# Bismarrck/tensoralloy

Hardware: AMD Instinct MI355X
Metric: atom-steps/sec (energy+forces), 4000-atom Ni rcut=6.5 A (higher is better)
Workload: dtype f64

## Files before the change

tensoralloy_amd/csrc/ta_api.hip:

```cpp
#include <hip/hip_runtime.h>

#include <algorithm>
#include <chrono>
#include <climits>
#include <cmath>
#include <cstdio>
#include <cstdlib>
#include <cstring>
#include <stdexcept>
#include <string>
#include <vector>

#include "ta_device.h"
#include "ta_internal.h"
#include "ta_md.h"
#include "ta_neb.h"
#include "ta_relax.h"

namespace ta {
size_t mlp_scratch_doubles(const MlpDev &mlp);
void launch_mlp_impl(const MlpDev &mlp, int activation, int ndim, const int32_t *atoms, int n_atoms,
                     const DeviceBatch &b, const Options &opt, double *scratch, hipStream_t s,
                     MlpLaunchInfo *info = nullptr);
size_t mlp_all_scratch_doubles(const MlpDev *mlps_host, int nel, const int32_t *elem_start);
// ... 204 lines not shown
  double rmax = 0.0;
  ta::SFParams sf;
  std::vector<ChunkPlan> chunks;
  std::vector<ChunkPlan> chunks_v2;
  bool use_v2 = false;
  ta::MlpDev *mlp_dev = nullptr;
  ta::MlpDev mlp[ta::kMaxElements];
  bool td = false, td_sommerfeld = false;
  int td_act = 0, td_K = 0;
  ta::MlpDev td_nets[3 * ta::kMaxElements];
  ta::MlpDev *td_dev = nullptr;
  std::vector<void *> model_allocs;
  ta::EamModel *eam = nullptr;
  ta::GrapModel *grap = nullptr;

  ta::HostPairs hp;
  ta::DeviceBatch db;
  bool have_batch = false;
  uint32_t last_want = 0;

  PinnedBuf stage_in, stage_out;
  DevBuf<char> inbuf;
  DevBuf<double> results;
  size_t o_blk = 0;
  int res_n_blk = 0;
  DevBuf<double> rec, part4, G, dEdG, g, wat, bpart, fown, benergy, mlp_scratch;
  DevBuf<double> td_T, td_u, td_s;
  DevBuf<unsigned long long> masks;
  DevBuf<uint32_t> job_word;
  DevBuf<int32_t> job_count;
  DevBuf<uint32_t> job_word_own;
  DevBuf<int32_t> job_count_own;
  bool triangles = true;
  bool tri_cells_ok = false;
  bool tri_cells_wide_ok = false;
  int last_bwd_variant = 0;
  ta::MlpLaunchInfo last_mlp_launch;
  DevBuf<int32_t> pair_start, seg_start, pair_i, pair_j, pair_shift, pair_rev;
  ta::NlGrid *d_grids = nullptr;
  DevBuf<int32_t> nl_wrap, nl_binid, nl_bin_count, nl_bin_start, nl_bin_cursor, nl_bin_atoms, nl_counts;
  DevBuf<unsigned long long> nl_stats, nl_zero;
  unsigned long long *nl_stats_ptr = nullptr;
  bool nl_sorted = false;
  bool nl_rev_done = false;
  bool nl_zero_clean = false;
  int64_t nl_zero_atoms = -1;
  int nl_zero_bins = -1;
  DevBuf<double> hvp_buf;
#ifdef TA_PHASE_STAMPS
  DevBuf<unsigned long long> stamp_buf;
#endif
  DevBuf<ta::NlRec> nl_recs;
  bool pairs_on_device = false;
  bool descriptors_valid = false;
  DevBuf<double> train_scratch, train_partial, train_grad, train_coeff;
  DevBuf<double> jvp_J, tan_dD, tan_dG, tan_dir;
  DevBuf<double> filt_scratch;
  bool jvp_valid = false;

  double skin = 0.0;
  double r_list = 0.0;
  std::vector<int32_t> keep_species;
  std::vector<int32_t> keep_natoms, keep_pbc;
  std::vector<double> ref_pos, ref_cells;
  size_t o_pos = 0, o_cells = 0, o_species = 0;
  DevBuf<int32_t> ex_pair_i, ex_pair_j, ex_pair_shift, ex_pair_rev, ex_pair_start, ex_pair_stop, ex_seg_start, ex_counts,
// ... 513 lines not shown
}

#ifdef TA_PHASE_STAMPS
static void dump_stamps(ta_context *h) {
  const std::string &path = h->opt.phase_stamps_out;
  if (path.empty() || !h->db.stamps || h->db.n_blk <= 0) return;
  const size_t n = (size_t)2 * h->db.n_blk * ta::kStampSlots;
  std::vector<unsigned long long> v(n);
  (void)hipStreamSynchronize(h->stream);
  (void)hipMemcpy(v.data(), h->db.stamps, n * sizeof(unsigned long long), hipMemcpyDeviceToHost);
  FILE *fp = std::fopen(path.c_str(), "w");
  if (!fp) return;
  for (int k = 0; k < 2; ++k)
    for (int b = 0; b < h->db.n_blk; ++b) {
      std::fprintf(fp, "%d %d", k, b);
      for (int q = 0; q < ta::kStampSlots; ++q)
        std::fprintf(fp, " %llu", v[((size_t)k * h->db.n_blk + b) * ta::kStampSlots + q]);
      std::fprintf(fp, "\n");
    }
  std::fclose(fp);
}
#endif

void launch_head(ta_context *h, const ta::DeviceBatch &db, hipStream_t s) {
  if (h->td)
    ta::launch_td_all(h->td_dev, h->td_nets, h->n_elements, h->td_K, h->td_act, h->activation,
                      h->td_sommerfeld ? 1 : 0, h->sf.ndim, db, h->opt.mlp_da_global, h->td_T.ptr, h->td_u.ptr, h->td_s.ptr,
                      h->mlp_scratch.ptr, s, &h->last_mlp_launch);
  else
    ta::launch_mlp_all(h->mlp_dev, h->mlp, h->n_elements, h->activation, h->sf.ndim, db, h->opt, h->mlp_scratch.ptr,
                       s, &h->last_mlp_launch);
}

void compute_impl(ta_context *h, uint32_t want, bool timed, double *slot_ms) {
  using namespace ta;
#ifdef TA_PHASE_STAMPS
  if (h->db.n_blk > 0) {
    h->stamp_buf.ensure((size_t)2 * h->db.n_blk * ta::kStampSlots + 8);
    h->db.stamps = h->stamp_buf.ptr;
    (void)hipMemsetAsync(h->db.stamps, 0, (size_t)2 * h->db.n_blk * ta::kStampSlots * sizeof(unsigned long long),
                         h->stream);
  }
#endif
  h->db.rec4 = nullptr;
  h->db.own_sums = 0;
  const DeviceBatch &db = h->db;
  hipStream_t s = h->stream;
  const bool need_forces = (want & (TA_WANT_FORCES | TA_WANT_VIRIAL)) != 0;
  auto begin = [&](int slot) {
    if (timed) HIP_CHECK(hipEventRecord(h->ev[2 * slot], s));
  };
  auto end = [&](int slot) {
    if (timed) HIP_CHECK(hipEventRecord(h->ev[2 * slot + 1], s));
  };
  bool used[TA_N_KERNEL_SLOTS] = {false};

  const bool has_mlp = h->kind == TA_MODEL_SF_MLP || h->kind == TA_MODEL_GRAP_MLP;
  if ((want & TA_WANT_REUSE_DESCRIPTORS) && has_mlp && h->descriptors_valid && !need_forces) {
    begin(TA_K_MLP);
    launch_head(h, db, s);
    end(TA_K_MLP);
    used[TA_K_MLP] = true;
  } else if (h->kind == TA_MODEL_SF_MLP) {
    h->db.rec4 = (h->sf.angular && h->use_v2 && !h->opt.full_records) ? h->db.rec : nullptr;
    if (!h->use_v2) {
      begin(TA_K_PAIR_GEOMETRY);
      launch_pair_geometry(h->sf, db, s);
      end(TA_K_PAIR_GEOMETRY);
      used[TA_K_PAIR_GEOMETRY] = true;
    }
    h->sf.ang_scale = h->use_v2 ? 1.0 : 0.5;
    const bool tri_cells = (h->relax_cell_on || h->md_baro_on) ? h->tri_cells_wide_ok : h->tri_cells_ok;
    const bool tri = h->use_v2 && h->triangles && tri_cells && h->n_elements == 1 && need_forces;
    h->db.job_word_own = (tri && h->db.job_count) ? h->job_word_own.ptr : nullptr;
    h->db.job_count_own = (tri && h->db.job_count) ? h->job_count_own.ptr : nullptr;
    h->last_bwd_variant = 0;
    const bool reduce_in_forward = h->sf.angular && h->use_v2;
    if (h->sf.angular) {
      begin(TA_K_G4_FORWARD);
      if (h->use_v2) {
        bool geometry = true;
        size_t left = h->chunks_v2.size();
        for (const ChunkPlan &cp : h->chunks_v2) {
          --left;
          launch_g4_forward_v2(h->sf, cp.ch, cp.ng, cp.nz, geometry, left == 0, db, h->opt, s);
          geometry = false;
        }
      } else
        for (const ChunkPlan &cp : h->chunks) launch_g4_forward(h->sf, cp.ch, cp.nb, cp.ng, cp.nz, db, s);
      end(TA_K_G4_FORWARD);
      used[TA_K_G4_FORWARD] = true;
    }
    if (!reduce_in_forward) {
      begin(TA_K_DESCRIPTOR_REDUCE);
      launch_descriptor_reduce(h->sf, db, s);
      end(TA_K_DESCRIPTOR_REDUCE);
      used[TA_K_DESCRIPTOR_REDUCE] = true;
    }
    begin(TA_K_MLP);
    launch_head(h, db, s);
    end(TA_K_MLP);
    used[TA_K_MLP] = true;
    if (need_forces) {
      begin(TA_K_BACKWARD);
      if (h->sf.angular) {
        bool first = true;
        if (h->use_v2)
          for (const ChunkPlan &cp : h->chunks_v2) {
            h->last_bwd_variant |= launch_backward_v2(h->sf, cp.ch, cp.ng, cp.nz, first, tri, db, h->opt, s);
            first = false;
          }
        else
          for (const ChunkPlan &cp : h->chunks) {
            launch_backward(h->sf, cp.ch, cp.nb, cp.ng, cp.nz, first, false, db, s);
            first = false;
          }
      } else {
        AngChunk dummy;
        std::memset(&dummy, 0, sizeof(dummy));
        launch_backward(h->sf, dummy, 1, 1, 1, true, true, db, s);
      }
// ... 283 lines not shown
  h->filtered = true;
}

bool cells_admit_triangles(double rmax, int32_t n_frames, const ta_frame *frames) {
  for (int f = 0; f < n_frames; ++f) {
    const double *c = frames[f].cell;
    const double vol = std::fabs(c[0] * (c[4] * c[8] - c[5] * c[7]) - c[1] * (c[3] * c[8] - c[5] * c[6]) +
                                 c[2] * (c[3] * c[7] - c[4] * c[6]));
    for (int k = 0; k < 3; ++k) {
      if (!frames[f].pbc[k]) continue;
      const double *u = c + 3 * ((k + 1) % 3), *v = c + 3 * ((k + 2) % 3);
      const double nx = u[1] * v[2] - u[2] * v[1], ny = u[2] * v[0] - u[0] * v[2], nz = u[0] * v[1] - u[1] * v[0];
      const double area = std::sqrt(nx * nx + ny * ny + nz * nz);
      if (!(vol > rmax * area)) return false;
    }
  }
  return true;
}

void set_frames_impl(ta_context *h, int32_t n_frames, const ta_frame *frames, ta_batch_info *info) {
  for (int f = 0; f < n_frames; ++f) {
    const ta_frame &fr = frames[f];
    if (fr.n_atoms < 0 || (fr.n_atoms > 0 && (!fr.species || !fr.positions)) || !fr.cell || !fr.pbc)
      throw std::invalid_argument("frame " + std::to_string(f) + ": null array");
  }
  const auto t_begin = std::chrono::steady_clock::now();
  if (h->upload_pending) {
    HIP_CHECK(hipStreamSynchronize(h->stream));
    h->upload_pending = false;
  }
  h->have_batch = false;
  h->descriptors_valid = false;
  h->jvp_valid = false;
  h->mirror_want = 0;
  h->filtered = false;
  h->db.slot_q = h->db.rev_super = h->db.rev_map = nullptr;
  h->db.pair_stop = nullptr;
  h->db.blk_groups = 0;
  h->db.n_blk_dev = nullptr;
  h->r_list = h->rmax + h->skin;
  h->tri_cells_ok = cells_admit_triangles(h->rmax, n_frames, frames);
  h->tri_cells_wide_ok = cells_admit_triangles(h->r_list, n_frames, frames);
  size_t N = 0;
  for (int f = 0; f < n_frames; ++f) N += (size_t)frames[f].n_atoms;
  if (N >= (1u << 30)) throw std::runtime_error("batch too large for 32-bit atom indices");
  const size_t F = (size_t)n_frames;
  const int nel = h->n_elements;
  auto align16 = [](size_t x) { return (x + 15) & ~(size_t)15; };
  const size_t o_pos = 0;
  const size_t o_cells = align16(o_pos + 3 * N * sizeof(double));
  const size_t o_grids = align16(o_cells + 9 * F * sizeof(double));
  const size_t o_species = align16(o_grids + F * sizeof(ta::NlGrid));
  const size_t o_foa = align16(o_species + N * sizeof(int32_t));
  const size_t o_astart = align16(o_foa + N * sizeof(int32_t));
  const size_t o_elem = align16(o_astart + (F + 1) * sizeof(int32_t));
  const size_t o_blk = align16(o_elem + N * sizeof(int32_t));
  auto align64 = [](size_t x) { return (x + 63) & ~(size_t)63; };
  const size_t total = align64(o_blk + (N + 2) * sizeof(int32_t)) + (N + 1) * sizeof(ta::BlockHeader);
  h->stage_in.ensure(total);
  h->inbuf.ensure(total);
  char *hb = h->stage_in.ptr;
  double *pos = reinterpret_cast<double *>(hb + o_pos);
  double *cells = reinterpret_cast<double *>(hb + o_cells);
  ta::NlGrid *grids = reinterpret_cast<ta::NlGrid *>(hb + o_grids);
  int32_t *species = reinterpret_cast<int32_t *>(hb + o_species);
  int32_t *foa = reinterpret_cast<int32_t *>(hb + o_foa);
// ... 252 lines not shown
}

int ta_set_skin(ta_handle h, double skin) {
  if (!h) return TA_ERR_INVALID;
  if (!(skin >= 0.0) || !std::isfinite(skin)) return fail(h, TA_ERR_INVALID, "skin must be a finite length >= 0");
  if (skin != h->skin) {
    h->skin = skin;
    h->have_batch = false;
    h->descriptors_valid = false;
  }
  return TA_OK;
}

int ta_update_positions(ta_handle h, const double *positions, const double *cells, int32_t *rebuilt) {
  if (!h || !positions) return fail(h, TA_ERR_INVALID, "null argument");
  if (h->ref_pos.empty() && h->keep_natoms.empty())
    return fail(h, TA_ERR_INVALID, "ta_update_positions called before ta_set_frames");
  return guarded(h, [&]() {
    const size_t N = h->keep_species.size(), F = h->keep_natoms.size();
    bool keep = h->have_batch && h->skin > 0.0;
    if (keep && cells) keep = std::memcmp(cells, h->ref_cells.data(), 9 * F * sizeof(double)) == 0;
    if (keep) {
      if (h->upload_pending) {
        HIP_CHECK(hipStreamSynchronize(h->stream));
        h->upload_pending = false;
      }
      double *stage = reinterpret_cast<double *>(h->stage_in.ptr + h->o_pos);
      std::memcpy(stage, positions, 3 * N * sizeof(double));
      staged_copy(h->db.pos, stage, 3 * N, false, h->opt, h->stream);
      h->upload_pending = true;
      if (h->filtered) apply_filter(h);
      h->descriptors_valid = false;
      h->jvp_valid = false;
      const double lim2 = 0.25 * h->skin * h->skin;
      const double *ref = h->ref_pos.data();
      for (size_t i = 0; i < N; ++i) {
        const double dx = positions[3 * i] - ref[3 * i], dy = positions[3 * i + 1] - ref[3 * i + 1],
                     dz = positions[3 * i + 2] - ref[3 * i + 2];
        const double d2 = dx * dx + dy * dy + dz * dz;
        if (!(d2 <= lim2)) {
          keep = false;
          break;
        }
      }
    }
    if (rebuilt) *rebuilt = keep ? 0 : 1;
    if (keep) {
      ++h->n_list_reuses;
      return;
    }
    rebuild_list(h, positions, cells);
    if (cells && h->relax_cell_on && h->relax_valid && F) {
      HIP_CHECK(hipMemcpy(h->relax_cell_h0.ptr, h->ref_cells.data(), 9 * F * sizeof(double), hipMemcpyHostToDevice));
      h->relax_cell_G_host.assign(9 * F, 0.0);
      for (size_t f = 0; f < F; ++f) h->relax_cell_G_host[9 * f] = h->relax_cell_G_host[9 * f + 4] = h->relax_cell_G_host[9 * f + 8] = 1.0;
      h->relax_cell_vel_host.assign(9 * F, 0.0);
    }
  });
}

int ta_list_stats(ta_handle h, int64_t *n_builds, int64_t *n_reuses) {
  if (!h) return TA_ERR_INVALID;
  if (n_builds) *n_builds = h->n_list_builds;
  if (n_reuses) *n_reuses = h->n_list_reuses;
  return TA_OK;
}
// ... 1311 lines not shown
    size_t scratch = 0, partial = 0;
    for (int e = 0; e < h->n_elements; ++e) {
      const int n_el = h->db.elem_start[e + 1] - h->db.elem_start[e];
      scratch = std::max(scratch, ta::mlp_grad_scratch_doubles(h->mlp[e], n_el));
      partial = std::max(partial, ta::mlp_grad_partial_doubles(h->mlp[e], n_el));
    }
    h->train_scratch.ensure(scratch + 8);
    h->train_partial.ensure(partial + 8);
    h->train_grad.ensure((size_t)total + 8);
    h->train_coeff.ensure(F + 8);
    if (F) HIP_CHECK(hipMemcpyAsync(h->train_coeff.ptr, frame_coeff, F * sizeof(double), hipMemcpyHostToDevice, s));
    size_t off = 0;
    for (int e = 0; e < h->n_elements; ++e) {
      const int n_el = h->db.elem_start[e + 1] - h->db.elem_start[e];
      ta::launch_mlp_grad(h->mlp[e], h->activation, h->sf.ndim, h->db.elem_atoms + h->db.elem_start[e], n_el,
                          h->db, h->train_coeff.ptr, h->train_scratch.ptr, h->train_partial.ptr,
                          h->train_grad.ptr + off, s);
      off += (size_t)ta::mlp_param_count(h->mlp[e]);
    }
    HIP_CHECK(hipGetLastError());
    HIP_CHECK(hipMemcpyAsync(grad, h->train_grad.ptr, (size_t)total * sizeof(double), hipMemcpyDeviceToHost, s));
    HIP_CHECK(hipStreamSynchronize(s));
  });
}

namespace {
void backward_only(ta_context *h) {
  using namespace ta;
  const DeviceBatch &db = h->db;
  hipStream_t s = h->stream;
  if (h->kind == TA_MODEL_SF_MLP) {
    if (h->sf.angular) {
      bool first = true;
      if (h->use_v2)
        for (const ChunkPlan &cp : h->chunks_v2) {
          launch_backward_v2(h->sf, cp.ch, cp.ng, cp.nz, first, false, db, h->opt, s);
          first = false;
        }
      else
        for (const ChunkPlan &cp : h->chunks) {
          launch_backward(h->sf, cp.ch, cp.nb, cp.ng, cp.nz, first, false, db, s);
          first = false;
        }
    } else {
      AngChunk dummy;
      std::memset(&dummy, 0, sizeof(dummy));
      launch_backward(h->sf, dummy, 1, 1, 1, true, true, db, s);
    }
  } else {
    launch_grap_backward(h->grap, db, s);
  }
}
void ensure_pair_jacobians(ta_context *h) {
  hipStream_t s = h->stream;
  const size_t N = (size_t)h->db.n_atoms, P = (size_t)h->db.n_pairs;
  const int D = h->sf.ndim;
  if (!h->descriptors_valid || !h->jvp_valid)
    compute_impl(h, TA_WANT_ENERGY, false, nullptr);
  if (h->jvp_valid) return;
  h->jvp_J.ensure((size_t)D * 4 * P + 8);
  for (int c = 0; c < D; ++c) {
    ta::launch_one_hot(h->db.dEdG, (int64_t)N, D, c, s);
    backward_only(h);
    if (P)
      HIP_CHECK(hipMemcpyAsync(h->jvp_J.ptr + (size_t)c * 4 * P, h->db.g, 4 * P * sizeof(double),
                               hipMemcpyDeviceToDevice, s));
  }
  HIP_CHECK(hipGetLastError());
  h->jvp_valid = true;
}
}

// ... 703 lines not shown
```

tensoralloy_amd/csrc/ta_device.h:

```cpp
#pragma once
#include <hip/hip_runtime.h>

#include <cstdint>
#include <type_traits>

#include "ta_options.h"
#include "tensoralloy_amd.h"

namespace ta {

constexpr int kMaxRadial = 64;
constexpr int kMaxElements = 8;
constexpr int kMaxBetaSlots = 3;
constexpr int kRecDoubles = 8;
constexpr int kMaxLayers = 8;
constexpr int kCapMin = 192;
constexpr int kCapMax = 1024;
constexpr int kMaxCentersPerBlock = 16;
constexpr int kMaxHd = 24;
constexpr int kStampSlots = 10;

struct SFParams {
  double rcut, acut;
  double inv_rc2, inv_ac2;
// ... 117 lines not shown
  int32_t ndim;
  uint32_t stride_nrad;
};
static_assert(sizeof(LaunchHead) == 64 && alignof(LaunchHead) == 64, "one line of the argument segment");
static_assert(std::is_trivially_copyable<LaunchHead>::value && std::is_standard_layout<LaunchHead>::value,
              "passed by value in the argument segment");
static_assert(4 * kCapMax < (1 << 16) && kMaxRadial < (1 << 8), "job_stride and n_rad share a word");

__host__ __device__ inline int triangle_owner_rank(uint32_t index_sum) {
#ifdef __HIP_DEVICE_COMPILE__
  const uint32_t h = __umul24(index_sum, 0x9E3779u);
#else
  const uint32_t h = index_sum * 0x9E3779u;
#endif
  return (int)(((h & 0xFFFFFFu) * 3u) >> 24);
}
__host__ __device__ inline bool owns_triangle(int32_t i, int32_t j, int32_t k) {
  return triangle_owner_rank((uint32_t)i + (uint32_t)j + (uint32_t)k) == (j < i ? 1 : 0) + (k < i ? 1 : 0);
}

#ifdef __HIPCC__
__device__ __forceinline__ int pair_stop_of(const DeviceBatch &b, int64_t i) {
  return b.pair_stop ? b.pair_stop[i] : b.pair_start[i + 1];
}
#endif

#ifdef __HIPCC__
__device__ __forceinline__ int pair_rev_of(const DeviceBatch &b, int q) {
  return b.slot_q ? b.rev_map[b.rev_super[b.slot_q[q]]] : b.pair_rev[q];
}
__device__ __forceinline__ const double2 *pair_geom(const DeviceBatch &b, size_t q) {
  return reinterpret_cast<const double2 *>(b.rec4 ? b.rec4 + 4 * q : b.rec + kRecDoubles * q);
}
#endif

struct MlpLayerDev {
  int k, n;
  int kp, np;
  double *w;
  double *wt;
  double *b;
  int act;
  int res;
};
struct MlpDev {
  int n_layers = 0;
  MlpLayerDev layer[kMaxLayers];
  double *xlo = nullptr, *xhi = nullptr;
  int max_np = 0, max_kp = 0;
};

struct MlpLaunchInfo {
  int family = 0;
  int threads = 0;
  int lh = 0;
  int nt = 0;
  int grid_x = 0, grid_y = 0;
  long long lds_bytes = 0;
  int da = 0;
};

void launch_pair_geometry(const SFParams &sf, const DeviceBatch &b, hipStream_t s);
void launch_g4_forward(const SFParams &sf, const AngChunk &ch, int nb, int ng, int nz,
                       const DeviceBatch &b, hipStream_t s);
void launch_descriptor_reduce(const SFParams &sf, const DeviceBatch &b, hipStream_t s);
void launch_mlp(const SFParams &sf, const MlpDev &mlp, int activation, int element,
                const DeviceBatch &b, hipStream_t s);
void launch_backward(const SFParams &sf, const AngChunk &ch, int nb, int ng, int nz,
                     bool first, bool radial_only, const DeviceBatch &b, hipStream_t s);
void launch_force_gather(const SFParams &sf, const DeviceBatch &b, int gather_w, hipStream_t s);
void launch_frame_reduce(const DeviceBatch &b, bool want_virial, double *mirror, int64_t n_tail, hipStream_t s);

size_t g4_lds_bytes(int nnl_max);

size_t v2_lds_bytes(bool backward, int cap, int n_local = 0, int nspec = 0, bool triangles = false);
int v2_job_stride(int cap);
void launch_g4_forward_v2(const SFParams &sf, const AngChunk &ch, int ng, int nz, bool geometry,
                          bool reduce, const DeviceBatch &b, const Options &opt, hipStream_t s);
int launch_backward_v2(const SFParams &sf, const AngChunk &ch, int ng, int nz, bool first, bool triangles,
                       const DeviceBatch &b, const Options &opt, hipStream_t s);

struct NlGrid {
  double h[9];
  double hinv[9];
  double lo[3];
  double inv_w[3];
  int32_t nb[3];
  int32_t pbc[3];
  int32_t bin_offset;
  int32_t pad_;
  int32_t m[3];
  int32_t ortho;
  double bw[3];
};
struct NlRec {
  double x, y, z;
  int32_t wx, wy, wz;
  int32_t j;
  int32_t sp;
  int32_t pad_;
};
struct NlWork {
  int32_t *wrap;
  int32_t *binid;
  int32_t *bin_count;
  int32_t *bin_start;
  int32_t *bin_cursor;
  int32_t *bin_atoms;
  NlRec *recs;
  int32_t *counts;
  int32_t *seg_start;
// ... 29 lines not shown
```

tensoralloy_amd/csrc/ta_kernels_v2.hip:

```cpp
#include <hip/hip_runtime.h>

#include <cstdio>
#include <cstdlib>
#include <stdexcept>
#include <type_traits>

#include "ta_device.h"
#include "ta_math.h"
#include "ta_reduce.h"

namespace ta {
namespace {

constexpr int kBlock = 256;
constexpr int kNF = 8;
constexpr int kNFf = 7;
constexpr int kSegW = 6;
constexpr int kOwnCtl = 60 + 2 * kMaxCentersPerBlock * kSegW;
constexpr int kJobCtlBytes = (kOwnCtl + 40) * 4;
__host__ __device__ inline int v2_pcols(int cap, int nspec) {
  return nspec >= 1 ? cap / 4 + kMaxCentersPerBlock * nspec : cap;
}
constexpr int kRingPad = 64;
constexpr int kRTab = 8;

#ifdef TA_LDS_PROBE
__device__ __forceinline__ bool kProbe(int flags, int bit) { return (flags >> bit) & 1; }
#else
__device__ __forceinline__ constexpr bool kProbe(int, int) { return false; }
#endif

#ifdef TA_PHASE_STAMPS
#define TA_STAMP(b, kernel, k)                                                                          \
  do {                                                                                                  \
    if ((b).stamps && threadIdx.x == 0)                                                                 \
      (b).stamps[((size_t)(kernel) * gridDim.x + blockIdx.x) * kStampSlots + (k)] = __builtin_amdgcn_s_memrealtime(); \
  } while (0)
#define TA_STAMP_ENTRY() const unsigned long long ta_t_start_ = __builtin_amdgcn_s_memrealtime()
#define TA_STAMP_HEADER(b, kernel, hd)                                                                  \
  do {                                                                                                  \
    if ((b).stamps && threadIdx.x == 0 && (hd).M >= 0) {                                                \
      unsigned long long *dst_ = (b).stamps + ((size_t)(kernel) * gridDim.x + blockIdx.x) * kStampSlots; \
      dst_[9] = __builtin_amdgcn_s_memrealtime();                                                       \
      dst_[8] = ta_t_start_;                                                                            \
    }                                                                                                   \
  } while (0)
#else
#define TA_STAMP(b, kernel, k) do {} while (0)
#define TA_STAMP_ENTRY() do {} while (0)
#define TA_STAMP_HEADER(b, kernel, hd) do {} while (0)
#endif

__device__ __forceinline__ void pin_head(const LaunchHead &h) {
  asm volatile("" ::"s"(h.blk_hdr), "s"(h.n_blk_dev), "s"(h.job_count), "s"(h.job_word), "s"(h.dEdG),
               "s"(h.pair_j), "s"(h.blk_groups), "s"(h.flags), "s"(h.ndim), "s"(h.stride_nrad));
// ... 94 lines not shown
  if constexpr (HD > 0) {
    double p = ch.hd[HD - 1], d = 0.0;
#pragma unroll
    for (int k = HD - 2; k >= 0; --k) {
      d = fma(d, u, p);
      p = fma(p, u, ch.hd[k]);
    }
    h = p;
    dh = d;
  } else {
    double fd, dfd;
    cutoff_u(sf.cutoff, u, fd, dfd);
    const double ed = ta_exp(-beta * u);
    h = ed * fd;
    dh = ed * (dfd - beta * fd);
  }
}
template <int HD>
__device__ __forceinline__ double hd_value(const SFParams &sf, const AngChunk &ch, double beta,
                                           double u) {
  if constexpr (HD > 0) {
    double p = ch.hd[HD - 1];
#pragma unroll
    for (int k = HD - 2; k >= 0; --k) p = fma(p, u, ch.hd[k]);
    return p;
  } else {
    return ta_exp(-beta * u) * cutoff_u_value(sf.cutoff, u);
  }
}

template <int HD>
__device__ __forceinline__ void stage(const SFParams &sf, const AngChunk &ch, double beta, const DeviceBatch &b,
                                      const Fields &f, const HeaderRegs &hd, const int32_t *pair_j, bool one_el,
                                      unsigned nthr, int geom = 0, bool forward = false, int *jidx = nullptr) {
  const int s0 = hd.s0, M = hd.M;
  for (int item = threadIdx.x; item < M; item += nthr) {
    double2 v0, v1, v2;
    int ci = 0, cbase = 0, cn = 0;
    if (geom || forward) centre_of(hd, item, ci, cbase, cn);
    const bool want_j = geom || jidx || !one_el;
    const int j = want_j ? (pair_j ? pair_j : b.pair_j)[s0 + item] : 0;
    const double spj = one_el ? 0.0 : (double)b.species[j];
    if (geom) {
      const int64_t p = (int64_t)s0 + item;
      const int i = hd.c0 + ci;
      const double *h = b.cells + 9 * (size_t)b.frame_of_atom[i];
      const double sx = (double)b.pair_shift[3 * p], sy = (double)b.pair_shift[3 * p + 1],
                   sz = (double)b.pair_shift[3 * p + 2];
      const double *ri = b.pos + 3 * (size_t)i, *rj = b.pos + 3 * (size_t)j;
      const double dx = (rj[0] - ri[0]) + (sx * h[0] + sy * h[3] + sz * h[6]);
      const double dy = (rj[1] - ri[1]) + (sx * h[1] + sy * h[4] + sz * h[7]);
      const double dz = (rj[2] - ri[2]) + (sx * h[2] + sy * h[5] + sz * h[8]);
      const double r2 = dx * dx + dy * dy + dz * dz + sf.eps;
      v0 = make_double2(dx, dy);
      v1 = make_double2(dz, r2);
      v2 = make_double2(1.0 / sqrt(r2), 0.0);
      if (b.rec4) {
        double2 *dst = reinterpret_cast<double2 *>(b.rec4 + 4 * (size_t)p);
        dst[0] = v0;
        dst[1] = v1;
      } else {
        double2 *dst = reinterpret_cast<double2 *>(b.rec + kRecDoubles * (size_t)p);
        dst[0] = v0;
        dst[1] = v1;
        dst[2] = v2;
        dst[3] = make_double2(0.0, 0.0);
      }
    } else if (b.rec4) {
      const double2 *src = reinterpret_cast<const double2 *>(b.rec4 + 4 * (size_t)(s0 + item));
      v0 = src[0];
      v1 = src[1];
      v2 = make_double2(1.0 / sqrt(v1.y), 0.0);
    } else {
      const double2 *src = reinterpret_cast<const double2 *>(b.rec + kRecDoubles * (size_t)(s0 + item));
      v0 = src[0];
      v1 = src[1];
      v2 = src[2];
    }
    f.xy[item] = v0;
    f.zr[item] = v1;
    if (forward) {
      const int k0 = 2 * cbase + (item - cbase);
      f.xf[k0] = f.xf[k0 + cn] = (float)v0.x;
      f.yf[k0] = f.yf[k0 + cn] = (float)v0.y;
      f.zf[k0] = f.zf[k0 + cn] = (float)v1.x;
    }
    const double u = v1.y * sf.inv_ac2;
    double H = 0.0, L = 0.0;
    if (u < 1.0) {
      if (forward) {
        H = hd_value<HD>(sf, ch, beta, u);
      } else {
        double dH;
        hd_eval<HD>(sf, ch, beta, u, H, dH);
        L = (H != 0.0) ? sf.two_inv_ac2 * dH / H : 0.0;
      }
    }
    f.ih[item] = make_double2(v2.x, H);
    if (jidx) jidx[item] = j;
    else if (forward) f.sp1[item] = spj;
    else f.gs[item] = make_double2(L, spj);
  }
  __syncthreads();
}

__device__ __forceinline__ unsigned long long partner_mask(const SFParams &sf, const Fields &f,
                                                           int base, int n, int a, int sc, int smax) {
  const int ring = 2 * base + a;
  const float ax = f.xf[ring], ay = f.yf[ring], az = f.zf[ring];
  const float lim = (float)(sf.acut * sf.acut) * 1.0001f;
  unsigned long long mask = 0ull;
  const int count = smax - sc + 1;
  typedef float f32x2 __attribute__((ext_vector_type(2)));
  const f32x2 ax2 = {ax, ax}, ay2 = {ay, ay}, az2 = {az, az};
  for (int g = 0; g < 4 && 16 * g < count; ++g) {
    const float *px = f.xf + ring + sc + 16 * g, *py = f.yf + ring + sc + 16 * g,
                *pz = f.zf + ring + sc + 16 * g;
    unsigned m = 0u;
#pragma unroll
    for (int k = 14; k >= 0; k -= 2) {
      const f32x2 vx = {px[k], px[k + 1]}, vy = {py[k], py[k + 1]}, vz = {pz[k], pz[k + 1]};
      const f32x2 ex = vx - ax2, ey = vy - ay2, ez = vz - az2;
      const f32x2 d2 = __builtin_elementwise_fma(ex, ex, __builtin_elementwise_fma(ey, ey, ez * ez));
      const float dhi = d2.y, dlo = d2.x;
      asm("v_cmp_lt_f32 vcc, %1, %2\n\tv_addc_co_u32 %0, vcc, %0, %0, vcc" : "+v"(m) : "v"(dhi), "v"(lim) : "vcc");
      asm("v_cmp_lt_f32 vcc, %1, %2\n\tv_addc_co_u32 %0, vcc, %0, %0, vcc" : "+v"(m) : "v"(dlo), "v"(lim) : "vcc");
    }
    mask |= (unsigned long long)m << (16 * g);
  }
  if (count < 64) mask &= (1ull << count) - 1ull;
  const int half = n >> 1;
  if (!(n & 1) && a >= half && half >= sc && half < sc + 64) mask &= ~(1ull << (half - sc));
  return mask;
}
// ... 306 lines not shown
  TA_STAMP_ENTRY();
  const int kCap = CAP > 0 ? CAP : b.cap;
  const int geom = flags & 1;
  if (b.n_blk_dev && (int)blockIdx.x >= *b.n_blk_dev) return;
  stagger(flags);
  extern __shared__ double lds[];
  const Fields f = carve(lds, kCap, true);
  const int slot = b.blk_groups > 0 ? 16 * ((int)blockIdx.x % b.blk_groups) + (int)blockIdx.x / b.blk_groups
                                    : (int)blockIdx.x;
  const BlockHeader *hp = b.blk_hdr + slot;
  const HeaderRegs hd = load_header(hp);
  TA_STAMP_HEADER(b, 0, hd);
  if (hd.ncent == 0) return;
  const int c0 = hd.c0, c1 = hd.c0 + hd.ncent;
  const int s0 = hd.s0, M = hd.M;
  const double beta = ch.beta[0];
  int *const cstart_w = reinterpret_cast<int *>(reinterpret_cast<char *>(lds) + v2_counter_offset(kCap)) + 40;
  if (threadIdx.x >= 40 && threadIdx.x < 40 + 17) cstart_w[threadIdx.x - 40] = hp->rel[threadIdx.x - 40];
  if (b.job_count) {
    char *raw = reinterpret_cast<char *>(lds);
    int *cnt = reinterpret_cast<int *>(raw + v2_counter_offset(kCap));
    if (threadIdx.x < 40) cnt[threadIdx.x] = 0;
    else if (threadIdx.x >= 64 && (int)threadIdx.x - 64 < (c1 - c0) * (NSPEC + 1)) {
      const int k = ((int)threadIdx.x - 64) / (NSPEC + 1), sg = ((int)threadIdx.x - 64) % (NSPEC + 1);
      cnt[60 + k * kSegW + sg] = NSPEC == 1 ? (int)hp->rel[k + sg]
                                            : b.seg_start[(size_t)(c0 + k) * (NSPEC + 1) + sg] - s0;
    }
    if (NSPEC == 1 && b.job_word_own && threadIdx.x < 20) cnt[kOwnCtl + threadIdx.x] = 0;
    double *P0 = reinterpret_cast<double *>(raw + v2_counter_offset(kCap) + kJobCtlBytes);
    for (int k = threadIdx.x; k < NSPEC * NG * NZ * v2_pcols(kCap, NSPEC); k += blockDim.x) P0[k] = 0.0;
  }
  int *jidx = (NSPEC == 1 && b.job_word_own && b.job_count) ? reinterpret_cast<int *>(f.sp1) : nullptr;
  TA_STAMP(b, 0, 0);
  stage<HD>(sf, ch, beta, b, f, hd, nullptr, NSPEC == 1, blockDim.x, geom, true, jidx);
  TA_STAMP(b, 0, 1);
  if (b.job_count && threadIdx.x == 0) {
    int *ctl = reinterpret_cast<int *>(reinterpret_cast<char *>(lds) + v2_counter_offset(kCap));
    const int *segl = ctl + 60;
    int *sslot = ctl + 60 + kMaxCentersPerBlock * kSegW;
    int acc = 0;
    for (int k = 0; k < c1 - c0; ++k)
      for (int sg = 0; sg <= NSPEC; ++sg) {
        sslot[k * kSegW + sg] = acc;
        if (sg < NSPEC) acc += (segl[k * kSegW + sg + 1] - segl[k * kSegW + sg] + 3) >> 2;
      }
  }

  auto run_item = [&](int item, bool have_mask, unsigned long long mask0, double *out, double *pacc, auto is_job) {
    constexpr bool kJob = decltype(is_job)::value;
    const int64_t p = (int64_t)s0 + item;
    int base, n;
    int pslot = item;
    unsigned own = 0u;
    int kbit = 0;
    uint32_t sij = 0u;
    int ic = 0, rij = 0;
    if constexpr (kJob) {
      const int *cstart = reinterpret_cast<const int *>(reinterpret_cast<const char *>(lds) + v2_counter_offset(kCap)) + 40;
      const int ci = job_centre((uint32_t)mask0);
      if (NSPEC == 1 && jidx) {
        ic = c0 + ci;
        const int j = jidx[item];
        sij = (uint32_t)ic + (uint32_t)j;
        rij = j < ic ? 1 : 0;
      }
      base = cstart[ci];
      n = cstart[ci + 1] - base;
// ... 123 lines not shown
            if (v != 0.0) atomicAdd(&pacc[(size_t)((sp * NG + ig) * NZ + iz) * v2_pcols(kCap, NSPEC) + pslot], v);
          } else if (out)
            out[(sp * NG + ig) * NZ + iz] = v;
          else
            b.part4[(size_t)(sp * sf.n_ang + c) * b.n_pairs + p] = v;
        }
    return own;
  };

  int item = threadIdx.x;
  const bool active = item < M;
  int ci_own = 0, base_own = 0, n_own = 0;
  if (active) centre_of(hd, item, ci_own, base_own, n_own);
  const bool one_pass = hd.one_pass;
  if (one_pass) {
    unsigned long long mask = 0ull;
    if (active) {
      const int64_t p = (int64_t)s0 + item;
      const int base = base_own;
      const int smax = (f.ih[item].y != 0.0) ? n_own / 2 : 0;
      if (smax > 0 && !(flags & (1 << 25))) mask = partner_mask(sf, f, base, n_own, item - base, 1, smax);
      if (b.masks && !b.job_count) b.masks[p] = mask;
    }
    TA_STAMP(b, 0, 2);
    if (b.job_count) {
      char *raw = reinterpret_cast<char *>(lds);
      JobLists jl = job_lists(f);
      jl.hist = reinterpret_cast<int *>(raw + v2_counter_offset(kCap));
      jl.start = jl.hist + 20;
      double *P = reinterpret_cast<double *>(raw + v2_counter_offset(kCap) + kJobCtlBytes);
      const int n_jobs = make_jobs(jl, active, item, ci_own, mask);
      TA_STAMP(b, 0, 3);
      const size_t jbase = (size_t)blockIdx.x * b.job_stride;
      if (threadIdx.x == 0) b.job_count[blockIdx.x] = n_jobs;
      for (int slot = threadIdx.x; slot < n_jobs; slot += blockDim.x) b.job_word[jbase + slot] = jl.word[slot];
      TA_STAMP(b, 0, 4);
      uint32_t swept[4] = {0u, 0u, 0u, 0u};
      unsigned owned[4] = {0u, 0u, 0u, 0u};
      if (!(flags & (1 << 27)))
        for (int r = 0; r * (int)blockDim.x < n_jobs; ++r) {
          const int slot = job_slot(r, threadIdx.x, blockDim.x);
          if (slot < n_jobs) {
            const uint32_t jw = jl.word[slot];
            const unsigned o = run_item(job_item(jw), true, jw, nullptr, P, std::true_type{});
            if (r < 4) {
              swept[r] = jw;
              owned[r] = o;
            }
          }
        }
      if (jidx)
        make_owned_jobs(jl.hist + kOwnCtl, jl.hist + kOwnCtl + 20, swept, owned, b.job_word_own + jbase,
                        b.job_count_own + blockIdx.x);
      __syncthreads();
      TA_STAMP(b, 0, 5);
      if (flags & 4) {
        assemble_flat<NSPEC, NG, NZ>(sf, ch, b, f, P, jl.hist + 60 + kMaxCentersPerBlock * kSegW, c0, c1, s0, item, active,
                                     (flags & (1 << 26)) != 0, kCap, blockDim.x);
        TA_STAMP(b, 0, 6);
        return;
      }
      if (active) {
        const int64_t p = (int64_t)s0 + threadIdx.x;
        const int ci = ci_own, sg = NSPEC == 1 ? 0 : (int)f.sp1[threadIdx.x];
        const int *segl = jl.hist + 60, *sslot = segl + kMaxCentersPerBlock * kSegW;
        const int rel = (int)threadIdx.x - segl[ci * kSegW + sg];
        const int pidx = sslot[ci * kSegW + sg] + (rel >> 2);
        const bool holds = (rel & 3) == 0;
// ... 501 lines not shown
      gz += b.g[4 * (size_t)p + 2];
    }
    b.g[4 * (size_t)p] = gx;
    b.g[4 * (size_t)p + 1] = gy;
    b.g[4 * (size_t)p + 2] = gz;
  }
  TA_STAMP(b, 1, 5);
}

template <class F>
struct first_param;
template <class A, class... As>
struct first_param<void (*)(A, As...)> {
  using type = A;
};
using BwdDefault = decltype(&backward_v2_kernel<1, 2, 2, 12, true, kCapMin, 5, true>);
static_assert(std::is_same<first_param<BwdDefault>::type, LaunchHead>::value, "LaunchHead leads the parameter list");

LaunchHead make_launch_head(const SFParams &sf, const DeviceBatch &b, int flags, bool own) {
  LaunchHead h;
  h.blk_hdr = b.blk_hdr;
  h.n_blk_dev = b.n_blk_dev;
  h.job_count = own ? b.job_count_own : b.job_count;
  h.job_word = own ? b.job_word_own : b.job_word;
  h.dEdG = b.dEdG;
  h.pair_j = b.pair_j;
  h.blk_groups = b.blk_groups;
  h.flags = flags;
  h.ndim = sf.ndim;
  h.stride_nrad = (uint32_t)b.job_stride | ((uint32_t)sf.n_rad << 16);
  return h;
}

template <int NSPEC, int NG, int NZ>
void fwd_t(const SFParams &sf, const AngChunk &ch, const DeviceBatch &b, int geom, int wpe, hipStream_t s) {
  const dim3 grid((unsigned)b.n_blk), block((unsigned)(b.cap < kBlock ? b.cap : kBlock));
  const size_t lds = v2_lds_bytes(false, b.cap, b.job_count ? NSPEC * NG * NZ : 0, NSPEC);
  if constexpr (NZ == 2) {
    if (ch.n_hd == 12 && ch.zeta_int[0] == 1 && ch.zeta_int[1] == 4) {
      if (b.cap == kCapMin) {
        if constexpr (NSPEC <= 2) {
          if (wpe != 5) {
            hipLaunchKernelGGL((g4_forward_v2_kernel<NSPEC, NG, NZ, 12, true, kCapMin, 6>), grid, block, lds, s, sf, ch,
                               b, geom);
            return;
          }
        }
        hipLaunchKernelGGL((g4_forward_v2_kernel<NSPEC, NG, NZ, 12, true, kCapMin>), grid, block, lds, s, sf, ch, b, geom);
      } else
        hipLaunchKernelGGL((g4_forward_v2_kernel<NSPEC, NG, NZ, 12, true, 0>), grid, block, lds, s, sf, ch, b, geom);
      return;
    }
    if (ch.n_hd == 16 && ch.zeta_int[0] == 1 && ch.zeta_int[1] == 4) {
      hipLaunchKernelGGL((g4_forward_v2_kernel<NSPEC, NG, NZ, 16, true, 0>), grid, block, lds, s, sf, ch, b, geom);
      return;
    }
  }
  if (ch.n_hd > 0 && ch.n_hd <= 16)
    hipLaunchKernelGGL((g4_forward_v2_kernel<NSPEC, NG, NZ, 16, false, 0>), grid, block, lds, s, sf, ch, b, geom);
  else if (ch.n_hd == 24)
    hipLaunchKernelGGL((g4_forward_v2_kernel<NSPEC, NG, NZ, 24, false, 0>), grid, block, lds, s, sf, ch, b, geom);
  else
    hipLaunchKernelGGL((g4_forward_v2_kernel<NSPEC, NG, NZ, 0, false, 0>), grid, block, lds, s, sf, ch, b, geom);
}
template <int NSPEC, int NG, int NZ>
void bwd_t(const SFParams &sf, const AngChunk &ch, const DeviceBatch &b, int first, bool tri, int wpe, int &variant,
           hipStream_t s) {
  const dim3 grid((unsigned)b.n_blk), block((unsigned)(b.cap < kBlock ? b.cap : kBlock));
  const size_t lds = v2_lds_bytes(true, b.cap);
  const LaunchHead head = make_launch_head(sf, b, first, false);
  const LaunchHead head_t = make_launch_head(sf, b, first, true);
  variant = 1;
  if constexpr (NZ == 2 && NSPEC == 1) {
    if (tri && (ch.n_hd == 12 || ch.n_hd == 16) && ch.zeta_int[0] == 1 && ch.zeta_int[1] == 4) {
      const size_t lds_t = v2_lds_bytes(true, b.cap, 0, 0, true);
      variant = 2;
      if (ch.n_hd == 12 && b.cap == kCapMin && wpe == 4)
        hipLaunchKernelGGL((backward_v2_kernel<1, NG, NZ, 12, true, kCapMin, 4, true>), grid, block, lds_t, s, head_t,
                           sf, ch, b);
      else if (ch.n_hd == 12 && b.cap == kCapMin)
        hipLaunchKernelGGL((backward_v2_kernel<1, NG, NZ, 12, true, kCapMin, 5, true>), grid, block, lds_t, s, head_t,
                           sf, ch, b);
      else if (ch.n_hd == 12)
        hipLaunchKernelGGL((backward_v2_kernel<1, NG, NZ, 12, true, 0, 5, true>), grid, block, lds_t, s, head_t,
                           sf, ch, b);
      else
        hipLaunchKernelGGL((backward_v2_kernel<1, NG, NZ, 16, true, 0, 5, true>), grid, block, lds_t, s, head_t,
                           sf, ch, b);
      return;
    }
  }
  if constexpr (NZ == 2) {
    if (ch.n_hd == 12 && ch.zeta_int[0] == 1 && ch.zeta_int[1] == 4) {
      if (b.cap == kCapMin) {
        if constexpr (NSPEC == 1) {
          if (wpe == 6) {
            hipLaunchKernelGGL((backward_v2_kernel<NSPEC, NG, NZ, 12, true, kCapMin, 6>), grid, block, lds, s,
                               head, sf, ch, b);
            return;
          }
        }
        hipLaunchKernelGGL((backward_v2_kernel<NSPEC, NG, NZ, 12, true, kCapMin>), grid, block, lds, s,
                           head, sf, ch, b);
      } else
        hipLaunchKernelGGL((backward_v2_kernel<NSPEC, NG, NZ, 12, true, 0>), grid, block, lds, s, head, sf, ch, b);
      return;
    }
// ... 38 lines not shown
      case 111: FN<1, 1, 1>(__VA_ARGS__); break;                  \
      case 112: FN<1, 1, 2>(__VA_ARGS__); break;                  \
      case 121: FN<1, 2, 1>(__VA_ARGS__); break;                  \
      case 122: FN<1, 2, 2>(__VA_ARGS__); break;                  \
      case 211: FN<2, 1, 1>(__VA_ARGS__); break;                  \
      case 212: FN<2, 1, 2>(__VA_ARGS__); break;                  \
      case 221: FN<2, 2, 1>(__VA_ARGS__); break;                  \
      case 222: FN<2, 2, 2>(__VA_ARGS__); break;                  \
      case 311: FN<3, 1, 1>(__VA_ARGS__); break;                  \
      case 312: FN<3, 1, 2>(__VA_ARGS__); break;                  \
      case 321: FN<3, 2, 1>(__VA_ARGS__); break;                  \
      case 322: FN<3, 2, 2>(__VA_ARGS__); break;                  \
      case 422: FN<4, 2, 2>(__VA_ARGS__); break;                  \
      case 522: FN<5, 2, 2>(__VA_ARGS__); break;                  \
      default:                                                    \
        throw std::domain_error("no second-generation angular kernel for this (species, gamma, zeta) shape"); \
    }                                                             \
  } while (0)
#endif

static int stagger_bits(const Options &opt, bool backward) {
#ifdef TA_PROBE_SWITCHES
  if (opt.debug_no_triples) return 1 << 24;
  if (opt.debug_skip >= 0) return opt.debug_skip << 24;
  return backward ? opt.stagger_bwd : opt.stagger_fwd;
#else
  (void)opt;
  (void)backward;
  return 0;
#endif
}

void launch_g4_forward_v2(const SFParams &sf, const AngChunk &ch, int ng, int nz, bool geometry,
                          bool reduce, const DeviceBatch &b, const Options &opt, hipStream_t s) {
  if (b.n_blk == 0) return;
  const int nspec = sf.n_elements;
  const int geom = (geometry ? 1 : 0) | (reduce ? 2 : 0) | ((geometry && reduce) ? 4 : 0) |
                   stagger_bits(opt, false);
  TA_DISPATCH_V2(fwd_t, sf, ch, b, geom, opt.fwd_wpe, s);
}

int launch_backward_v2(const SFParams &sf, const AngChunk &ch, int ng, int nz, bool first, bool triangles,
                       const DeviceBatch &b, const Options &opt, hipStream_t s) {
  if (b.n_blk == 0) return 0;
  const int nspec = sf.n_elements;
  const int f = (first ? 1 : 0) | stagger_bits(opt, true);
  int variant = 0;
  TA_DISPATCH_V2(bwd_t, sf, ch, b, f, triangles, opt.bwd_wpe, variant, s);
  return variant;
}

}
```

Measured before the change: 38.36 million.

## Skip unused full job-list writes and stream pair records with buffer stores

The angular forward kernel no longer writes the full job-word list when the triangle backward kernel will consume only the owned-job list; it marks job_count as -1 instead. The fallback non-triangle backward path recomputes the forward first when that list is missing. Pair geometry records are now written after staging, through raw buffer stores with a cache-policy bit, which is meant to cut write traffic and cache pollution. This adds a validity flag that must be reset whenever positions or frames change, and a lazy recompute that costs time on the paths that need it.

```diff
diff --git a/tensoralloy_amd/csrc/ta_api.hip b/tensoralloy_amd/csrc/ta_api.hip
--- a/tensoralloy_amd/csrc/ta_api.hip
+++ b/tensoralloy_amd/csrc/ta_api.hip
@@ -260,6 +260,7 @@
   DevBuf<uint32_t> job_word_own;
   DevBuf<int32_t> job_count_own;
   bool triangles = true;
+  bool full_jobs_valid = false;
   bool tri_cells_ok = false;
   bool tri_cells_wide_ok = false;
   int last_bwd_variant = 0;
@@ -839,6 +840,20 @@
                        s, &h->last_mlp_launch);
 }
 
+void forward_v2_launches(ta_context *h, bool tri) {
+  using namespace ta;
+  bool unread = tri && h->db.job_word_own && h->db.job_count_own && h->db.job_count;
+  for (const ChunkPlan &cp : h->chunks_v2) unread = unread && v2_backward_takes_triangles(h->sf, cp.ch, cp.ng, cp.nz);
+  bool geometry = true;
+  size_t left = h->chunks_v2.size();
+  for (const ChunkPlan &cp : h->chunks_v2) {
+    --left;
+    launch_g4_forward_v2(h->sf, cp.ch, cp.ng, cp.nz, geometry, left == 0, unread, h->db, h->opt, h->stream);
+    geometry = false;
+  }
+  h->full_jobs_valid = !unread;
+}
+
 void compute_impl(ta_context *h, uint32_t want, bool timed, double *slot_ms) {
   using namespace ta;
 #ifdef TA_PHASE_STAMPS
@@ -885,15 +900,9 @@
     const bool reduce_in_forward = h->sf.angular && h->use_v2;
     if (h->sf.angular) {
       begin(TA_K_G4_FORWARD);
-      if (h->use_v2) {
-        bool geometry = true;
-        size_t left = h->chunks_v2.size();
-        for (const ChunkPlan &cp : h->chunks_v2) {
-          --left;
-          launch_g4_forward_v2(h->sf, cp.ch, cp.ng, cp.nz, geometry, left == 0, db, h->opt, s);
-          geometry = false;
-        }
-      } else
+      if (h->use_v2)
+        forward_v2_launches(h, tri);
+      else
         for (const ChunkPlan &cp : h->chunks) launch_g4_forward(h->sf, cp.ch, cp.nb, cp.ng, cp.nz, db, s);
       end(TA_K_G4_FORWARD);
       used[TA_K_G4_FORWARD] = true;
@@ -1243,6 +1252,7 @@
   h->have_batch = false;
   h->descriptors_valid = false;
   h->jvp_valid = false;
+  h->full_jobs_valid = false;
   h->mirror_want = 0;
   h->filtered = false;
   h->db.slot_q = h->db.rev_super = h->db.rev_map = nullptr;
@@ -1561,6 +1571,7 @@
       if (h->filtered) apply_filter(h);
       h->descriptors_valid = false;
       h->jvp_valid = false;
+      h->full_jobs_valid = false;
       const double lim2 = 0.25 * h->skin * h->skin;
       const double *ref = h->ref_pos.data();
       for (size_t i = 0; i < N; ++i) {
@@ -2938,12 +2949,13 @@
   if (h->kind == TA_MODEL_SF_MLP) {
     if (h->sf.angular) {
       bool first = true;
-      if (h->use_v2)
+      if (h->use_v2) {
+        if (db.job_count && !h->full_jobs_valid) forward_v2_launches(h, false);
         for (const ChunkPlan &cp : h->chunks_v2) {
           launch_backward_v2(h->sf, cp.ch, cp.ng, cp.nz, first, false, db, h->opt, s);
           first = false;
         }
-      else
+      } else
         for (const ChunkPlan &cp : h->chunks) {
           launch_backward(h->sf, cp.ch, cp.nb, cp.ng, cp.nz, first, false, db, s);
           first = false;
diff --git a/tensoralloy_amd/csrc/ta_device.h b/tensoralloy_amd/csrc/ta_device.h
--- a/tensoralloy_amd/csrc/ta_device.h
+++ b/tensoralloy_amd/csrc/ta_device.h
@@ -173,7 +173,23 @@
 __device__ __forceinline__ const double2 *pair_geom(const DeviceBatch &b, size_t q) {
   return reinterpret_cast<const double2 *>(b.rec4 ? b.rec4 + 4 * q : b.rec + kRecDoubles * q);
 }
-#endif
+struct WtSlice {
+  __amdgpu_buffer_rsrc_t rsrc;
+};
+__device__ __forceinline__ WtSlice wt_slice(void *base, uint32_t bytes) {
+  WtSlice s;
+  s.rsrc = __builtin_amdgcn_make_buffer_rsrc(base, 0, (int)bytes, 0x00020000);
+  return s;
+}
+__device__ __forceinline__ void wt_store16(const WtSlice &s, uint32_t byte_offset, double2 v) {
+  typedef uint32_t u32x4 __attribute__((ext_vector_type(4)));
+  const u32x4 w = {(uint32_t)__double2loint(v.x), (uint32_t)__double2hiint(v.x), (uint32_t)__double2loint(v.y),
+                   (uint32_t)__double2hiint(v.y)};
+  __builtin_amdgcn_raw_buffer_store_b128(w, s.rsrc, (int)byte_offset, 0, 16);
+}
+#endif
+constexpr size_t kWtMaxBytes = (size_t)32 << 20;
+inline bool wt_handover(const DeviceBatch &b) { return 32 * (size_t)b.n_pairs <= kWtMaxBytes; }
 
 struct MlpLayerDev {
   int k, n;
@@ -217,7 +233,8 @@
 size_t v2_lds_bytes(bool backward, int cap, int n_local = 0, int nspec = 0, bool triangles = false);
 int v2_job_stride(int cap);
 void launch_g4_forward_v2(const SFParams &sf, const AngChunk &ch, int ng, int nz, bool geometry,
-                          bool reduce, const DeviceBatch &b, const Options &opt, hipStream_t s);
+                          bool reduce, bool full_list_unread, const DeviceBatch &b, const Options &opt, hipStream_t s);
+bool v2_backward_takes_triangles(const SFParams &sf, const AngChunk &ch, int ng, int nz);
 int launch_backward_v2(const SFParams &sf, const AngChunk &ch, int ng, int nz, bool first, bool triangles,
                        const DeviceBatch &b, const Options &opt, hipStream_t s);
 
diff --git a/tensoralloy_amd/csrc/ta_kernels_v2.hip b/tensoralloy_amd/csrc/ta_kernels_v2.hip
--- a/tensoralloy_amd/csrc/ta_kernels_v2.hip
+++ b/tensoralloy_amd/csrc/ta_kernels_v2.hip
@@ -21,6 +21,15 @@
 __host__ __device__ inline int v2_pcols(int cap, int nspec) {
   return nspec >= 1 ? cap / 4 + kMaxCentersPerBlock * nspec : cap;
 }
+#ifndef TA_HANDOVER_REC_LATE
+#define TA_HANDOVER_REC_LATE 1
+#endif
+#ifndef TA_HANDOVER_SKIP_LIST
+#define TA_HANDOVER_SKIP_LIST 1
+#endif
+#ifndef TA_HANDOVER_WT_REC
+#define TA_HANDOVER_WT_REC 1
+#endif
 constexpr int kRingPad = 64;
 constexpr int kRTab = 8;
 
@@ -181,8 +190,39 @@
 template <int HD>
 __device__ __forceinline__ void stage(const SFParams &sf, const AngChunk &ch, double beta, const DeviceBatch &b,
                                       const Fields &f, const HeaderRegs &hd, const int32_t *pair_j, bool one_el,
-                                      unsigned nthr, int geom = 0, bool forward = false, int *jidx = nullptr) {
+                                      unsigned nthr, int geom = 0, bool forward = false, int *jidx = nullptr,
+                                      bool wt = false) {
   const int s0 = hd.s0, M = hd.M;
+#if TA_HANDOVER_WT_REC
+  const WtSlice wt_rec = wt_slice(b.rec4 ? b.rec4 + 4 * (size_t)s0 : nullptr, (geom && b.rec4) ? 32u * (uint32_t)M : 0u);
+#else
+  (void)wt;
+#endif
+  auto store_record = [&](int item, double2 v0, double2 v1, double2 v2) {
+#ifdef TA_PROBE_NO_HANDOVER
+    (void)item; (void)v0; (void)v1; (void)v2;
+#else
+    const int64_t p = (int64_t)s0 + item;
+    if (b.rec4) {
+#if TA_HANDOVER_WT_REC
+      if (wt) {
+        wt_store16(wt_rec, 32u * (uint32_t)item, v0);
+        wt_store16(wt_rec, 32u * (uint32_t)item + 16u, v1);
+        return;
+      }
+#endif
+      double2 *dst = reinterpret_cast<double2 *>(b.rec4 + 4 * (size_t)p);
+      dst[0] = v0;
+      dst[1] = v1;
+    } else {
+      double2 *dst = reinterpret_cast<double2 *>(b.rec + kRecDoubles * (size_t)p);
+      dst[0] = v0;
+      dst[1] = v1;
+      dst[2] = v2;
+      dst[3] = make_double2(0.0, 0.0);
+    }
+#endif
+  };
   for (int item = threadIdx.x; item < M; item += nthr) {
     double2 v0, v1, v2;
     int ci = 0, cbase = 0, cn = 0;
@@ -204,17 +244,9 @@
       v0 = make_double2(dx, dy);
       v1 = make_double2(dz, r2);
       v2 = make_double2(1.0 / sqrt(r2), 0.0);
-      if (b.rec4) {
-        double2 *dst = reinterpret_cast<double2 *>(b.rec4 + 4 * (size_t)p);
-        dst[0] = v0;
-        dst[1] = v1;
-      } else {
-        double2 *dst = reinterpret_cast<double2 *>(b.rec + kRecDoubles * (size_t)p);
-        dst[0] = v0;
-        dst[1] = v1;
-        dst[2] = v2;
-        dst[3] = make_double2(0.0, 0.0);
-      }
+#if !TA_HANDOVER_REC_LATE
+      store_record(item, v0, v1, v2);
+#endif
     } else if (b.rec4) {
       const double2 *src = reinterpret_cast<const double2 *>(b.rec4 + 4 * (size_t)(s0 + item));
       v0 = src[0];
@@ -249,6 +281,9 @@
     if (jidx) jidx[item] = j;
     else if (forward) f.sp1[item] = spj;
     else f.gs[item] = make_double2(L, spj);
+#if TA_HANDOVER_REC_LATE
+    if (geom) store_record(item, v0, v1, v2);
+#endif
   }
   __syncthreads();
 }
@@ -621,7 +656,7 @@
   }
   int *jidx = (NSPEC == 1 && b.job_word_own && b.job_count) ? reinterpret_cast<int *>(f.sp1) : nullptr;
   TA_STAMP(b, 0, 0);
-  stage<HD>(sf, ch, beta, b, f, hd, nullptr, NSPEC == 1, blockDim.x, geom, true, jidx);
+  stage<HD>(sf, ch, beta, b, f, hd, nullptr, NSPEC == 1, blockDim.x, geom, true, jidx, (flags & 16) != 0);
   TA_STAMP(b, 0, 1);
   if (b.job_count && threadIdx.x == 0) {
     int *ctl = reinterpret_cast<int *>(reinterpret_cast<char *>(lds) + v2_counter_offset(kCap));
@@ -811,8 +846,16 @@
       const int n_jobs = make_jobs(jl, active, item, ci_own, mask);
       TA_STAMP(b, 0, 3);
       const size_t jbase = (size_t)blockIdx.x * b.job_stride;
-      if (threadIdx.x == 0) b.job_count[blockIdx.x] = n_jobs;
-      for (int slot = threadIdx.x; slot < n_jobs; slot += blockDim.x) b.job_word[jbase + slot] = jl.word[slot];
+#if defined(TA_PROBE_NO_HANDOVER)
+      const bool skip_full = true;
+#elif TA_HANDOVER_SKIP_LIST
+      const bool skip_full = (flags & 8) && jidx;
+#else
+      const bool skip_full = false;
+#endif
+      if (threadIdx.x == 0) b.job_count[blockIdx.x] = skip_full ? -1 : n_jobs;
+      if (!skip_full)
+        for (int slot = threadIdx.x; slot < n_jobs; slot += blockDim.x) b.job_word[jbase + slot] = jl.word[slot];
       TA_STAMP(b, 0, 4);
       uint32_t swept[4] = {0u, 0u, 0u, 0u};
       unsigned owned[4] = {0u, 0u, 0u, 0u};
@@ -1380,8 +1423,13 @@
   return h;
 }
 
+bool takes_triangles(int nspec, int nz, const AngChunk &ch) {
+  return nspec == 1 && nz == 2 && (ch.n_hd == 12 || ch.n_hd == 16) && ch.zeta_int[0] == 1 && ch.zeta_int[1] == 4;
+}
+
 template <int NSPEC, int NG, int NZ>
 void fwd_t(const SFParams &sf, const AngChunk &ch, const DeviceBatch &b, int geom, int wpe, hipStream_t s) {
+  if (!(b.job_word_own && b.job_count && takes_triangles(NSPEC, NZ, ch))) geom &= ~8;
   const dim3 grid((unsigned)b.n_blk), block((unsigned)(b.cap < kBlock ? b.cap : kBlock));
   const size_t lds = v2_lds_bytes(false, b.cap, b.job_count ? NSPEC * NG * NZ : 0, NSPEC);
   if constexpr (NZ == 2) {
@@ -1420,7 +1468,7 @@
   const LaunchHead head_t = make_launch_head(sf, b, first, true);
   variant = 1;
   if constexpr (NZ == 2 && NSPEC == 1) {
-    if (tri && (ch.n_hd == 12 || ch.n_hd == 16) && ch.zeta_int[0] == 1 && ch.zeta_int[1] == 4) {
+    if (tri && takes_triangles(NSPEC, NZ, ch)) {
       const size_t lds_t = v2_lds_bytes(true, b.cap, 0, 0, true);
       variant = 2;
       if (ch.n_hd == 12 && b.cap == kCapMin && wpe == 4)
@@ -1525,16 +1573,24 @@
 }
 
 void launch_g4_forward_v2(const SFParams &sf, const AngChunk &ch, int ng, int nz, bool geometry,
-                          bool reduce, const DeviceBatch &b, const Options &opt, hipStream_t s) {
+                          bool reduce, bool full_list_unread, const DeviceBatch &b, const Options &opt, hipStream_t s) {
   if (b.n_blk == 0) return;
   const int nspec = sf.n_elements;
   const int geom = (geometry ? 1 : 0) | (reduce ? 2 : 0) | ((geometry && reduce) ? 4 : 0) |
-                   stagger_bits(opt, false);
+                   (full_list_unread ? 8 : 0) | (wt_handover(b) ? 16 : 0) | stagger_bits(opt, false);
   TA_DISPATCH_V2(fwd_t, sf, ch, b, geom, opt.fwd_wpe, s);
+}
+
+bool v2_backward_takes_triangles(const SFParams &sf, const AngChunk &ch, int ng, int nz) {
+  (void)ng;
+  return takes_triangles(sf.n_elements, nz, ch);
 }
 
 int launch_backward_v2(const SFParams &sf, const AngChunk &ch, int ng, int nz, bool first, bool triangles,
                        const DeviceBatch &b, const Options &opt, hipStream_t s) {
+#ifdef TA_PROBE_NO_HANDOVER
+  throw std::domain_error("TA_PROBE_NO_HANDOVER build: the forward kernel left no pair records, no forces");
+#endif
   if (b.n_blk == 0) return 0;
   const int nspec = sf.n_elements;
   const int f = (first ? 1 : 0) | stagger_bits(opt, true);
```

New measurement: 38.98 million (median of 6 runs). 1.02x the previous value.
